# DaehwanKimLab/centrifuge

Hardware: NVIDIA H100
Metric: reads/sec (100 bp SE classification) (higher is better)
Workload: dtype u64

## Files before the change

centrifuge_b200/capi.py:

```python
import ctypes as C
import os

import numpy as np

HERE = os.path.dirname(os.path.abspath(__file__))
LIB_PATH = os.path.join(HERE, "libcfb200.so")

CFB_UID_NONE = 0xFFFFFFFF
REC_DTYPE = np.dtype([("taxid", "<u8"), ("score", "<u4"), ("hitlen", "<u4"), ("uid", "<u4"), ("pad", "<u4")])

_lib = None


class CfbError(RuntimeError):
    pass


class IndexInfo(C.Structure):
    _fields_ = [("len", C.c_uint64), ("num_sides", C.c_uint64), ("n_seqs", C.c_uint64), ("n_tax_nodes", C.c_uint64),
                ("n_boundaries", C.c_uint64), ("line_rate", C.c_int32), ("off_rate", C.c_int32), ("ftab_chars", C.c_int32),
                ("sample_bytes", C.c_int32), ("compressed", C.c_int32), ("device", C.c_int32), ("device_bytes", C.c_uint64)]


class IndexTables(C.Structure):
# ... 289 lines not shown

    def search_iter_stats(self):
        out = (C.c_uint64 * 8)()
        _ck(lib().cfb_ctx_search_iter_stats(self.h, out))
        names = ["warp_iters", "lane_requests", "consumer_paths", "restart_paths", "task_iters", "clk_head", "clk_wait", "clk_tail"]
        return dict(zip(names, [int(x) for x in out]))

    def score_stats(self):
        out = (C.c_uint64 * 23)()
        _ck(lib().cfb_ctx_score_stats(self.h, out))
        v = [int(x) for x in out]
        names = ["units", "rows", "distinct_ids", "reduce_units", "reduce_rounds", "warps", "warps_global"]
        d = dict(zip(names, v[:7]))
        d["rows_hist"], d["distinct_ids_hist"] = v[7:15], v[15:23]
        return d

    def long_stats(self):
        out = (C.c_uint64 * 4)()
        _ck(lib().cfb_ctx_long_stats(self.h, out))
        return dict(zip(["units", "bases", "segment_searches", "researched"], [int(x) for x in out]))

    def counters(self):
        out = (C.c_uint64 * 8)()
        _ck(lib().cfb_ctx_counters(self.h, out))
        names = ["units", "partial_searches", "ftab_probes", "sides_search", "walk_steps", "rows_resolved", "lf_steps", "ext_searches"]
        return dict(zip(names, [int(x) for x in out]))

    def launches(self):
        n = C.c_uint64()
        _ck(lib().cfb_ctx_kernel_launches(self.h, C.byref(n)))
# ... 253 lines not shown
```

centrifuge_b200/csrc/cf_logic.h:

```cpp
#ifndef CF_LOGIC_H_
#define CF_LOGIC_H_

#include <stdint.h>

#ifdef __CUDACC__
#define CFB_HD __host__ __device__ __forceinline__
#define CFB_HDN __host__ __device__
#else
#define CFB_HD inline
#define CFB_HDN inline
#endif

namespace cfb {

static const uint64_t kOff = 0xffffffffffffffffull;
static const uint64_t kUnk = 0xfffffffffffffffeull;
static const uint32_t kBwNone = 0xffffffffu;

struct alignas(16) SeqInfo {
	uint64_t taxid;
	int32_t  pid;
	uint32_t flags;
};
static const uint32_t kSeqExcluded = 1u;
// ... 30 lines not shown

struct Params {
	uint32_t khits, min_hitlen, ihits, increment;
	uint32_t tree_traverse, class_rank_slot;
};

struct HitRec { uint64_t top, bot; uint32_t bwoff, len; };

static const uint64_t kRowMask = (1ull << 40) - 1ull, kRowStart = 1ull << 63, kRowSameTs = 1ull << 58;

struct Counters {
	unsigned long long units, partial_searches, ftab_probes, sides_search, walk_steps, rows_resolved, lf_steps, ext_searches;
	unsigned long long req_rank16, req_ftab2, req_ftabk, req_walk8, req_ftabd;
	unsigned long long r16_w1, r16_w2_4, r16_w5, w8_try_row, w8_ok_row, w8_try_range, w8_ok_range, w8_ok_w5;
	unsigned long long it_warp, it_lane_req, it_consumers, it_restarts, it_task, clk_head, clk_wait, clk_tail;
	unsigned long long sc_units, sc_rows, sc_nmap, sc_reduce, sc_rounds, sc_warps, sc_warps_global;
	unsigned long long sc_rows_hist[8], sc_nmap_hist[8];
};

CFB_HD int popc64(uint64_t x) {
#ifdef __CUDA_ARCH__
	return __popcll(x);
#else
	return __builtin_popcountll(x);
#endif
}
CFB_HD uint32_t ctz32(uint32_t x) {
#ifdef __CUDA_ARCH__
	return (uint32_t)(__ffs(x) - 1);
#else
// ... 787 lines not shown
```

centrifuge_b200/csrc/cf_multi.cuh:

```cuda
#include <dlfcn.h>
#include <nccl.h>

extern "C" int cfb_ctx_count_records(cfb_ctx* c, int on) {
	if(!c) return fail(CFB_EINVAL, "null ctx");
	CK(cudaSetDevice(c->ix->device));
	if(on) { int rc = counts_init(c); if(rc) return rc; }
	c->fold_records = on != 0;
	return CFB_OK;
}
extern "C" int cfb_counts_taxids(cfb_ctx* c, uint64_t* taxid, uint64_t cap, uint64_t* n) {
	if(!c || !n) return fail(CFB_EINVAL, "null argument");
	CK(cudaSetDevice(c->ix->device));
	int rc = counts_init(c); if(rc) return rc;
	*n = c->cnt.n;
	if(taxid) { if(cap < c->cnt.n) return fail(CFB_EINVAL, "cfb_counts_taxids: buffer too small"); memcpy(taxid, c->cnt.h_taxid.data(), (size_t)c->cnt.n * 8); }
	return CFB_OK;
}
extern "C" int cfb_counts_reset(cfb_ctx* c) {
	if(!c) return fail(CFB_EINVAL, "null ctx");
	CK(cudaSetDevice(c->ix->device));
	if(!c->cnt.ready) return CFB_OK;
	CK(cudaDeviceSynchronize());
	CK(cudaMemset(c->cnt.total.p, 0, 3ull * c->cnt.n * 8)); CK(cudaMemset(c->cnt.global.p, 0, 3ull * c->cnt.n * 8));
	c->cnt.reduced = false;
// ... 153 lines not shown
	if(!c || !out) return fail(CFB_EINVAL, "null argument");
	CK(cudaSetDevice(c->ix->device));
	Counters h; CK(cudaMemcpy(&h, c->d_ctr, sizeof h, cudaMemcpyDeviceToHost));
	out[0] = h.it_warp; out[1] = h.it_lane_req; out[2] = h.it_consumers; out[3] = h.it_restarts; out[4] = h.it_task;
	out[5] = h.clk_head; out[6] = h.clk_wait; out[7] = h.clk_tail;
	return CFB_OK;
}
extern "C" int cfb_ctx_score_stats(cfb_ctx* c, uint64_t out[23]) {
	if(!c || !out) return fail(CFB_EINVAL, "null argument");
	CK(cudaSetDevice(c->ix->device));
	Counters h; CK(cudaMemcpy(&h, c->d_ctr, sizeof h, cudaMemcpyDeviceToHost));
	out[0] = h.sc_units; out[1] = h.sc_rows; out[2] = h.sc_nmap; out[3] = h.sc_reduce; out[4] = h.sc_rounds; out[5] = h.sc_warps; out[6] = h.sc_warps_global;
	for(int i = 0; i < 8; i++) { out[7 + i] = h.sc_rows_hist[i]; out[15 + i] = h.sc_nmap_hist[i]; }
	return CFB_OK;
}

__device__ __forceinline__ uint64_t gmix(uint64_t x) { x += 0x9E3779B97F4A7C15ull; x = (x ^ (x >> 30)) * 0xBF58476D1CE4E5B9ull; x = (x ^ (x >> 27)) * 0x94D049BB133111EBull; return x ^ (x >> 31); }
template <int W, int ILP>
__global__ void __launch_bounds__(128) k_gather_probe(const unsigned long long* __restrict__ a, uint64_t n, uint32_t iters, unsigned long long* sink) {
	const uint64_t tid = (uint64_t)blockIdx.x * blockDim.x + threadIdx.x;
	uint64_t h = gmix(tid * 0x2545F4914F6CDD1Dull + 1), acc = 0;
	for(uint32_t it = 0; it < iters; it++) {
		unsigned long long v[ILP][W];
		#pragma unroll
		for(int k = 0; k < ILP; k++) {
			h = gmix(h + k);
			const uint64_t u = h % n;
			if(W == 2) { const ulonglong2 q = __ldg(reinterpret_cast<const ulonglong2*>(a) + u); v[k][0] = q.x; v[k][W - 1] = q.y; }
			else v[k][0] = __ldg(a + u);
		}
// ... 42 lines not shown
```

centrifuge_b200/csrc/cfb200.cu:

```cuda
#include "../../include/cfb200.h"
#include "cf_index.h"
#include "cf_kernels.cuh"
#include <cub/cub.cuh>

#include <algorithm>
#include <atomic>
#include <mutex>
#include <thread>
#include <fcntl.h>
#include <unistd.h>
#include <cstdarg>
#include <cstdio>
#include <cstring>
#include <set>
#include <string>
#include <vector>

using namespace cfb;

enum { M_DONE = 0, M_FTAB = 1, M_LF = 2, M_NEED = 3, M_FTABK = 4, M_TASK = 5 };

struct SearchArgs {
	IndexView v; Params p; BatchView b;
	HitRec* hits; uint32_t* nhits; uint32_t cap;
// ... 557 lines not shown
		u.rdlen[r] = len; fw[r] = a.b.bases + a.b.off[m][unit]; tpos[r] = t0;
		const uint32_t raw[2] = {a.nhits[t0], a.nhits[t0 + 1]};
		for(int st = 0; st < 2; st++) {
			if(raw[st] & kListRegen) {
				const uint32_t slot = raw[st] & 0x3fffffffu;
				u.L[r][st] = a.regen + (size_t)slot * a.full_cap; u.n[r][st] = a.regen_n[slot]; found[r][st] = 0;
			} else {
				u.L[r][st] = a.hits + (t0 + st) * a.cap; u.n[r][st] = min(nh_stored(raw[st]), a.cap); found[r][st] = nh_found(raw[st]);
			}
		}
		for(int st = 0; st < 2; st++) if(list_dropped(raw, st)) u.n[r][st] = 0;
	}
	return u.n_mates > 0;
}

template <int MINB, bool EMIT_ONLY>
__global__ void __launch_bounds__(128, MINB) k_prep(const UnitArgs a) {
	const uint32_t unit = blockIdx.x * blockDim.x + threadIdx.x;
	const bool live = unit < a.b.n_units;
	UnitHits u; const uint8_t* fw[2]; uint32_t found[2][2]; size_t tpos[2];
	uint64_t rows = 0; bool have = false;
	if(live && (have = load_unit(a, unit, u, fw, found, tpos))) {
		if(EMIT_ONLY) { CountRows cr(a.p, u); for_each_visit(a.p, u, cr); rows = cr.rows; }
		else {
			Counters local; Counters* lc = nullptr;
			if(a.ctr) { memset(&local, 0, sizeof local); lc = &local; }
			if(!a.keep_short) for(int r = 0; r < u.n_mates; r++) {
				for(int st = 0; st < 2; st++) {
					if(!list_needs_regen(u.n[r][st], u.n[r][st ^ 1], found[r][st])) continue;
					const unsigned long long slot = atomicAdd(a.regen_ctr, 1ull);
					if(slot >= a.regen_slots) { atomicExch(a.overflow, 4u); continue; }
					HitRec* L = a.regen + (size_t)slot * a.full_cap;
					const uint32_t n = a.v.cr ? search_strand_dev<true>(a.v, a.p, fw[r], u.rdlen[r], st, L, a.full_cap)
					                          : search_strand_dev<false>(a.v, a.p, fw[r], u.rdlen[r], st, L, a.full_cap);
					if(n > a.full_cap) atomicExch(a.overflow, 1u);
					u.L[r][st] = L; u.n[r][st] = min(n, a.full_cap);
					a.regen_n[slot] = u.n[r][st]; a.nhits[tpos[r] + st] = kListRegen | (uint32_t)slot;
				}
			}
			for(int r = 0; r < u.n_mates; r++) {
				for(int st = 0; st < 2; st++) {
					if(!list_needs_exact_ranges(a.p, u.L[r][st], u.n[r][st], u.n[r][st ^ 1])) continue;
					for(uint32_t i = 0; i < u.n[r][st]; i++) {
						HitRec& h = u.L[r][st][i];
						if(h.top != kUnk) continue;
						HitRec t; uint32_t nc; bool dn;
						partial_search_scalar(a.v, fw[r], u.rdlen[r], st, h.bwoff, t, nc, dn, nullptr);
						h.top = t.top; h.bot = t.bot;
					}
				}
			}
			for(int r = 0; r < u.n_mates; r++) post_search(a.v, a.p, fw[r], u.rdlen[r], u.L[r][0], u.n[r][0], u.L[r][1], u.n[r][1], lc);
			SortAndCount sc(a.p, u);
			for_each_visit(a.p, u, sc);
// ... 3 lines not shown
				if(local.ext_searches) {
					atomicAdd(&a.ctr->ext_searches, local.ext_searches); atomicAdd(&a.ctr->partial_searches, local.partial_searches);
					atomicAdd(&a.ctr->ftab_probes, local.ftab_probes); atomicAdd(&a.ctr->sides_search, local.sides_search); atomicAdd(&a.ctr->lf_steps, local.lf_steps);
				}
			}
		}
		if(rows > 0xFFFFFFFFull) rows = 0xFFFFFFFFull;
	}
	const unsigned lane = threadIdx.x & 31;
	uint64_t incl = rows;
	for(int d = 1; d < 32; d <<= 1) { const uint64_t t = __shfl_up_sync(0xffffffffu, incl, d); if((int)lane >= d) incl += t; }
	const uint64_t warp_total = __shfl_sync(0xffffffffu, incl, 31);
	unsigned long long base = 0;
	if(lane == 31 && warp_total) base = atomicAdd(a.row_total, (unsigned long long)warp_total);
	base = __shfl_sync(0xffffffffu, base, 31);
	if(!live) return;
	const uint64_t off = base + incl - rows;
	a.nrows[unit] = (uint32_t)rows; a.row_off[unit] = off;
	if(rows && off + rows <= a.rows_cap) { EmitRows er(a.p, u, a.rows + off); for_each_visit(a.p, u, er); }
}

static const int kScoreThreads = 128;
static const uint32_t kScorePool = 232;
static const uint32_t kNoSlot = 0xffffffffu;
__device__ __forceinline__ uint32_t log2_bucket(uint64_t x) { const uint32_t b = 63u - (uint32_t)__clzll((long long)x); return b < 7u ? b : 7u; }
template <int MINB, bool COUNT>
__global__ void __launch_bounds__(kScoreThreads, MINB) k_score(const UnitArgs a) {
	__shared__ Entry s_map[kScorePool];
	__shared__ uint32_t s_used;
	if(threadIdx.x == 0) s_used = 0;
	__syncthreads();
	const uint32_t unit = blockIdx.x * blockDim.x + threadIdx.x;
	const unsigned lane = threadIdx.x & 31;
	const bool valid = unit < a.b.n_units;
// ... 159 lines not shown
			if(src < 0) break;
			chars |= (uint64_t)src << (2 * nv);
			row = next;
		}
		if(gl == 0) out[idx] = (row & kWalkRowMask) | (chars << 40) | ((uint64_t)nv << 56);
	}
}

__global__ void __launch_bounds__(256) k_lookup(const ResolveArgs a) {
	uint64_t n = *a.total; if(n > a.rows_cap) return;
	const uint64_t i = (uint64_t)blockIdx.x * blockDim.x + threadIdx.x;
	const uint64_t stride = (uint64_t)gridDim.x * blockDim.x;
	for(uint64_t k = i; k < n; k += stride) { const uint64_t r = a.rows[k] & kRowMask; a.ids[k] = a.v.rtab32 ? __ldg(a.v.rtab32 + r) : (uint32_t)__ldg(a.v.rtab16 + r); }
}

__global__ void __launch_bounds__(128) k_compact(uint32_t n_units, const uint64_t* row_off, const uint64_t* out_off,
                                                 const OutRec* sparse, OutRec* dense, uint32_t* rec_off32, uint64_t dense_cap, unsigned int* overflow) {
	const uint32_t unit = blockIdx.x * blockDim.x + threadIdx.x;
	if(unit > n_units) return;
	if(unit == n_units) { rec_off32[unit] = (uint32_t)out_off[unit]; return; }
	const uint64_t o = out_off[unit], n = out_off[unit + 1] - o;
	rec_off32[unit] = (uint32_t)o;
	if(o + n > dense_cap) { if(n) atomicExch(overflow, 3u); return; }
	const uint64_t src = row_off[unit];
	for(uint64_t i = 0; i < n; i++) dense[o + i] = sparse[src + i];
}

static const uint32_t kSegLen = 4096;
static_assert(kLongUnitLen == CFB_LONG_UNIT_LEN && kMaxMateLen == CFB_MAX_MATE_LEN, "cf_logic.h and cfb200.h disagree on the read length limits");
struct LongTask { uint64_t hoff, soff; uint32_t unit, mate, len, nseg; };
struct LongUnit { uint32_t unit, task0, ntask, pad; };
struct LongArgs {
	IndexView v; Params p; BatchView b;
	const LongTask* tasks; uint32_t ntasks; const LongUnit* units; uint32_t nunits; uint64_t nsegs;
	HitRec* seg; uint32_t* sn; uint32_t* sexit;
	HitRec* hits; uint32_t* nh;
	uint32_t* nrows; uint64_t* roff; uint32_t* hl;
	unsigned long long* stats;
	UnitArgs u;
};
// ... 385 lines not shown
}
extern "C" void cfb_params_default(cfb_params* p) {
	if(!p) return;
	memset(p, 0, sizeof *p); p->khits = 5; p->min_hitlen = 22; p->tree_traverse = 1; p->class_rank_slot = 0;
}

static const int kSlots = 17;

struct Slot {
	cudaStream_t st = nullptr;
	cudaEvent_t ev[6] = {nullptr, nullptr, nullptr, nullptr, nullptr, nullptr};
	HBuf<uint8_t> h_bases; HBuf<uint64_t> h_off; HBuf<uint32_t> h_len; HBuf<uint8_t> h_flags;
	DBuf<uint8_t> d_bases; DBuf<uint64_t> d_off; DBuf<uint32_t> d_len; DBuf<uint8_t> d_flags;
	HBuf<uint64_t> h_words; DBuf<uint64_t> d_words, d_npos, d_woff; DBuf<uint32_t> d_wlen;
	DBuf<uint64_t> pk; DBuf<uint32_t> nm;
	DBuf<HitRec> hits; DBuf<uint32_t> nhits; DBuf<HitRec> regen; DBuf<uint32_t> regen_n; uint64_t regen_slots = 0; uint32_t full_cap = 0; DBuf<uint32_t> nrows; DBuf<uint64_t> row_off; DBuf<uint64_t> bsum;
	DBuf<uint64_t> rows; DBuf<uint32_t> ids; DBuf<Entry> entries; DBuf<TaxCnt> tcs; DBuf<OutRec> sparse;
	DBuf<uint32_t> nout; DBuf<uint64_t> out_off; DBuf<uint8_t> scan_tmp; DBuf<OutRec> dense; DBuf<uint32_t> rec_off32;
	DBuf<unsigned long long> scal;
	HBuf<unsigned long long> h_scal;
	HBuf<OutRec> h_recs; HBuf<uint32_t> h_rec_off;
	DBuf<unsigned long long> cnt;
	bool folded = false, is_text = false, commit_pending = false;
	BatchView bv; uint64_t n_units = 0, n_bases = 0; uint32_t maxlen = 0, cap = 0; uint64_t rows_cap = 0, dense_cap = 0;
	bool pending = false, reran = false;
	bool want_host = false; uint64_t d2h_recs = 0;
	struct LongH { uint64_t unit; uint32_t len[2]; uint8_t fl; };
	std::vector<LongH> longs; uint64_t win_first = 0; uint32_t nlong_win = 0;
	HBuf<LongTask> h_ltask; HBuf<LongUnit> h_lunit; DBuf<LongTask> d_ltask; DBuf<LongUnit> d_lunit;
	DBuf<HitRec> lseg, lhits; DBuf<uint32_t> lsn, lsexit, lnh, lnrows, lhl; DBuf<uint64_t> lroff; DBuf<uint8_t> flags_short; DBuf<unsigned long long> lstats;
	uint64_t lhit_slots = 0, lsegs = 0; uint32_t lntasks = 0, lmaxlen = 0;
	void release() {
		h_bases.release(); h_off.release(); h_len.release(); h_flags.release(); d_bases.release(); d_off.release(); d_len.release(); d_flags.release();
		h_words.release(); d_words.release(); d_npos.release(); d_woff.release(); d_wlen.release();
		pk.release(); nm.release(); hits.release(); nhits.release(); regen.release(); regen_n.release(); nrows.release(); row_off.release(); bsum.release(); rows.release(); ids.release(); entries.release(); tcs.release();
		sparse.release(); nout.release(); out_off.release(); scan_tmp.release(); dense.release(); rec_off32.release(); scal.release(); h_scal.release(); h_recs.release(); h_rec_off.release(); cnt.release();
		h_ltask.release(); h_lunit.release(); d_ltask.release(); d_lunit.release(); lseg.release(); lhits.release(); lsn.release(); lsexit.release(); lnh.release();
		lnrows.release(); lhl.release(); lroff.release(); flags_short.release(); lstats.release();
		for(int i = 0; i < 6; i++) if(ev[i]) cudaEventDestroy(ev[i]);
		if(st) cudaStreamDestroy(st);
	}
};

struct cfb_dbatch { int slot; uint64_t n_units; };
struct TextCtx;
static void text_release(cfb_ctx*);
static void comm_release(cfb_ctx*);

struct CountsCtx {
	bool ready = false;
	std::vector<uint64_t> h_taxid; DBuf<uint64_t> d_taxid; uint32_t n = 0;
	DBuf<unsigned long long> total, global; bool reduced = false;
	void release() { d_taxid.release(); total.release(); global.release(); }
};

struct cfb_ctx {
	const cfb_index* ix = nullptr;
	IndexView view; Params prm;
	DBuf<uint64_t> d_host; DBuf<SeqInfo> d_seqs;
	Slot slots[kSlots];
	Counters* d_ctr = nullptr; int count = 0;
	uint64_t launches = 0;
	int resolve_blocks = 0;
	cfb_dbatch resident; bool resident_used = false;
	double rec_ratio = 2.0;
	uint64_t rows_cap0 = 0;
	TextCtx* text = nullptr;
	CountsCtx cnt; bool fold_records = false;
// ... 92 lines not shown
	*out = c;
	return CFB_OK;
}
extern "C" int cfb_ctx_slots(const cfb_ctx*) { return kSlots - 1; }
extern "C" int cfb_ctx_kernel_launches(const cfb_ctx* c, uint64_t* n) { if(!c || !n) return CFB_EINVAL; *n = c->launches; return CFB_OK; }

static int counts_init(cfb_ctx* c) {
	CountsCtx& k = c->cnt;
	if(k.ready) return CFB_OK;
	const HostIndex& h = c->ix->h;
	std::set<uint64_t> sp; sp.insert(0); sp.insert(1);
	for(size_t i = 0; i < h.nodes.size(); i++) sp.insert(h.nodes[i].taxid);
	sp.insert(h.seq_taxid.begin(), h.seq_taxid.end());
	k.h_taxid.assign(sp.begin(), sp.end()); k.n = (uint32_t)k.h_taxid.size();
	CK(k.d_taxid.ensure(k.n + 1)); CK(cudaMemcpy(k.d_taxid.p, k.h_taxid.data(), (size_t)k.n * 8, cudaMemcpyHostToDevice));
	CK(k.total.ensure(3ull * k.n)); CK(cudaMemset(k.total.p, 0, 3ull * k.n * 8));
	CK(k.global.ensure(3ull * k.n)); CK(cudaMemset(k.global.p, 0, 3ull * k.n * 8));
	k.ready = true;
	return CFB_OK;
}

struct FoldArgs {
	const uint64_t* sp_taxid; uint32_t n_sp;
	const uint32_t* rec_off; const OutRec* recs; uint32_t n_units; int32_t n_mates; uint32_t khits;
	const uint32_t* len[2]; const uint8_t* flags;
	unsigned long long* sp;
};
__device__ __forceinline__ int find_slot(const uint64_t* a, uint32_t n, uint64_t key) {
	uint32_t lo = 0, hi = n;
	while(lo < hi) { const uint32_t mid = (lo + hi) >> 1; if(a[mid] < key) lo = mid + 1; else hi = mid; }
	return (lo < n && a[lo] == key) ? (int)lo : -1;
}
__global__ void __launch_bounds__(128) k_fold_counts(const FoldArgs a) {
	const uint32_t u = blockIdx.x * 128 + threadIdx.x;
	const bool live = u < a.n_units;
	int first_slot = -1; uint32_t num = 1; bool qualifies = false;
	if(live) {
		const uint32_t r0 = a.rec_off[u], r1 = a.rec_off[u + 1];
		if(r1 == r0) { first_slot = find_slot(a.sp_taxid, a.n_sp, 0); qualifies = true; }
		else {
			uint32_t best = 0, ties = 0;
			for(uint32_t k = r0; k < r1; k++) { const uint32_t sc = a.recs[k].score; if(sc > best || k == r0) { best = sc; ties = 1; } else if(sc == best) ties++; }
			num = ties < a.khits ? ties : a.khits;
			const uint32_t fl = a.flags ? a.flags[u] : 3u;
			int64_t max_score = 0;
			if(fl & 1u) { const int64_t L = a.len[0][u]; max_score += L > 15 ? (L - 15) * (L - 15) : 0; }
			if(a.n_mates == 2 && (fl & 2u)) { const int64_t L = a.len[1][u]; max_score += L > 15 ? (L - 15) * (L - 15) : 0; }
			qualifies = (int64_t)best >= max_score;
			uint32_t taken = 0;
			for(uint32_t k = r0; k < r1 && taken < num; k++) {
				if(a.recs[k].score != best) continue;
				const int slot = find_slot(a.sp_taxid, a.n_sp, a.recs[k].taxid);
				if(taken == 0) first_slot = slot; else if(slot >= 0) atomicAdd(a.sp + slot, 1ull);
				taken++;
			}
		}
	}
	const int key = live ? first_slot : -1;
	const uint32_t peers = __match_any_sync(0xffffffffu, key);
	if(key >= 0) {
		const uint32_t uniq = __popc(__ballot_sync(peers, num == 1) & peers);
		const uint32_t obs = __popc(__ballot_sync(peers, num == 1 && qualifies) & peers);
		if((uint32_t)(__ffs(peers) - 1) == (threadIdx.x & 31u)) {
			atomicAdd(a.sp + key, (unsigned long long)__popc(peers));
			if(uniq) atomicAdd(a.sp + a.n_sp + key, (unsigned long long)uniq);
			if(obs) atomicAdd(a.sp + 2ull * a.n_sp + key, (unsigned long long)obs);
		}
	}
}
__global__ void k_cnt_commit(const unsigned long long* slot_sp, unsigned long long* total, uint32_t n) {
	const uint32_t i = blockIdx.x * blockDim.x + threadIdx.x;
	if(i < n) { const unsigned long long v = slot_sp[i]; if(v) atomicAdd(total + i, v); }
}

static int long_oom(const Slot& s, cudaError_t e, const char* what) {
	cudaGetLastError();
	uint64_t bases = 0; uint32_t mx = 0;
	for(const Slot::LongH& l : s.longs) { bases += (uint64_t)l.len[0] + l.len[1]; mx = std::max(mx, std::max(l.len[0], l.len[1])); }
	return fail(CFB_ENOMEM, "no device memory for %s of a batch with %zu long units (%llu bases, the longest read %u bases): %s", what,
	            s.longs.size(), (unsigned long long)bases, mx, cudaGetErrorString(e));
}
#define CKL(call, what) do { cudaError_t e_ = (call); if(e_ != cudaSuccess) { if(!s.longs.empty()) return long_oom(s, e_, what); CK(e_); } } while(0)

static int mate_too_long(uint64_t n, int m, const uint32_t* L) {
// ... 192 lines not shown
	BatchView sb = s.bv;
	if(s.nlong_win) sb.flags = s.flags_short.p;
	const uint32_t ublocks = (uint32_t)((n + 127) / 128);
	const uint64_t scan_blocks = (n + kScanBlock * kScanPer - 1) / (kScanBlock * kScanPer);
	if(n == 0) return CFB_OK;
	const SearchKernel search = search_kernel(s.maxlen, c->count, c->view.cr != nullptr);
	const bool keep_short = search == k_search_long<true> || search == k_search_long<false> || search == k_search_long<false, true> || c->prm.min_hitlen < kLongLen || c->keep_short;
	if(stage == 0) {
		if(s.cap == 0) {
			s.full_cap = s.maxlen / 4 + 8;
			s.cap = keep_short ? s.full_cap : s.maxlen / kLongLen + 2;
		}
		CK(s.hits.ensure(ntasks * s.cap)); CK(s.nhits.ensure(ntasks));
		if(!keep_short) {
			s.regen_slots = std::max<uint64_t>(s.regen_slots, c->regen_slots0 ? c->regen_slots0 : std::max<uint64_t>(ntasks / 32, 1024));
			CK(s.regen.ensure(s.regen_slots * s.full_cap)); CK(s.regen_n.ensure(s.regen_slots));
			CK(cudaMemsetAsync(s.scal.p + 6, 0, sizeof(unsigned long long), s.st));
		}
		const uint32_t W = (s.maxlen + 31) / 32 + 1;
		CK(s.pk.ensure(ntasks * W + 2)); CK(s.nm.ensure(ntasks * W + 2)); CK(s.nrows.ensure(n)); CK(s.row_off.ensure(n + 1));
		CK(s.bsum.ensure(scan_blocks + 1)); CK(s.nout.ensure(n + 1)); CK(s.out_off.ensure(n + 1)); CK(s.rec_off32.ensure(n + 1));
		s.rows_cap = std::max<uint64_t>(s.rows_cap, c->rows_cap0 ? c->rows_cap0 : std::max<uint64_t>(n * 12, 4096));
	}
	if(s.nlong_win) {
		CKL(s.rows.ensure(s.rows_cap), "the rows"); CKL(s.ids.ensure(s.rows_cap), "the rows"); CKL(s.entries.ensure(s.rows_cap), "the hit maps");
		CKL(s.tcs.ensure(s.rows_cap), "the hit maps"); CKL(s.sparse.ensure(s.rows_cap), "the records"); CKL(s.dense.ensure(s.rows_cap), "the records");
		CKL(s.lhl.ensure(s.rows_cap), "the rows");
	}
	CK(s.rows.ensure(s.rows_cap)); CK(s.ids.ensure(s.rows_cap)); CK(s.entries.ensure(s.rows_cap)); CK(s.tcs.ensure(s.rows_cap)); CK(s.sparse.ensure(s.rows_cap));
	s.dense_cap = s.rows_cap; CK(s.dense.ensure(s.dense_cap));
	CK(cudaMemsetAsync(s.scal.p, 0, 4 * sizeof(unsigned long long), s.st));
// ... 13 lines not shown
		SearchArgs sa; sa.v = c->view; sa.p = c->prm; sa.b = sb; sa.hits = s.hits.p; sa.nhits = s.nhits.p; sa.cap = s.cap;
		const uint32_t W = (s.maxlen + 31) / 32 + 1;
		sa.pk = s.pk.p; sa.nm = s.nm.p; sa.W = W; sa.keep_short = keep_short ? 1u : 0u;
		{ PackArgs pa; pa.b = sb; pa.pk = s.pk.p; pa.nm = s.nm.p; pa.W = W;
		  k_pack<<<(unsigned)((ntasks * W + 127) / 128), 128, 0, s.st>>>(pa); c->launches++; }
		sa.task_ctr64 = s.scal.p + 0; sa.ntasks = (uint32_t)ntasks; sa.overflow = (unsigned int*)(s.scal.p + 2); sa.ctr = ctr;
		int occ = 1;
		CK(cudaOccupancyMaxActiveBlocksPerMultiprocessor(&occ, search, kSearchThreads, 0));
		const uint64_t resident = (uint64_t)c->ix->sm_count * (uint64_t)std::max(occ, 1);
		const uint64_t warps = resident * (kSearchThreads / 32);
		sa.chunk = (uint32_t)std::min<uint64_t>(std::max<uint64_t>(ntasks / (warps * 4), 32), 256);
		const int blocks = (int)std::min<uint64_t>(resident, (ntasks + kSearchThreads - 1) / kSearchThreads);
		search<<<blocks, kSearchThreads, 0, s.st>>>(sa);
		c->launches++;
		if(time_it) CK(cudaEventRecord(s.ev[1], s.st));
		k_prep<8, false><<<ublocks, 128, 0, s.st>>>(ua); c->launches++;
	} else {
		if(time_it) CK(cudaEventRecord(s.ev[1], s.st));
		k_prep<8, true><<<ublocks, 128, 0, s.st>>>(ua); c->launches++;
	}
	LongArgs la;
	if(s.nlong_win) {
		la.v = c->view; la.p = c->prm; la.b = s.bv; la.tasks = s.d_ltask.p; la.ntasks = s.lntasks; la.units = s.d_lunit.p; la.nunits = s.nlong_win;
		la.nsegs = s.lsegs; la.seg = s.lseg.p; la.sn = s.lsn.p; la.sexit = s.lsexit.p; la.hits = s.lhits.p; la.nh = s.lnh.p;
		la.nrows = s.lnrows.p; la.roff = s.lroff.p; la.hl = s.lhl.p; la.stats = s.lstats.p; la.u = ua;
		const unsigned ub = (s.nlong_win + 31) / 32;
		if(stage == 0) {
			if(s.lntasks) {
				if(c->count == 1) k_long_join<true><<<(2 * s.lntasks + 127) / 128, 128, 0, s.st>>>(la);
				else {
// ... 13 lines not shown
	if((c->view.rtab16 || c->view.rtab32) && c->count != 1) k_lookup<<<c->ix->sm_count * 8, 256, 0, s.st>>>(ra);
	else if(c->view.cr) { if(c->count) k_resolve_c<true, false, true><<<c->resolve_blocks, kSearchThreads, 0, s.st>>>(ra); else k_resolve_c<false, false, true><<<c->resolve_blocks, kSearchThreads, 0, s.st>>>(ra); }
	else if(c->count) k_resolve_c<true, false><<<c->resolve_blocks, kSearchThreads, 0, s.st>>>(ra);
	else k_resolve_c<false, false><<<c->resolve_blocks, kSearchThreads, 0, s.st>>>(ra);
	c->launches++;
	if(time_it) CK(cudaEventRecord(s.ev[3], s.st));
	if(ctr) k_score<12, true><<<ublocks, kScoreThreads, 0, s.st>>>(ua);
	else k_score<12, false><<<ublocks, kScoreThreads, 0, s.st>>>(ua);
	if(s.nlong_win) { k_long_score<<<(s.nlong_win + 127) / 128, 128, 0, s.st>>>(la); c->launches++; }
	size_t scan_bytes = 0;
	CK(cub::DeviceScan::ExclusiveScan(nullptr, scan_bytes, s.nout.p, s.out_off.p, cub::Sum(), (uint64_t)0, (int)(n + 1), s.st));
	CK(s.scan_tmp.ensure(scan_bytes));
	CK(cudaMemsetAsync(s.nout.p + n, 0, sizeof(uint32_t), s.st));
	CK(cub::DeviceScan::ExclusiveScan(s.scan_tmp.p, scan_bytes, s.nout.p, s.out_off.p, cub::Sum(), (uint64_t)0, (int)(n + 1), s.st));
	CK(cudaMemcpyAsync(s.scal.p + 4, s.out_off.p + n, sizeof(uint64_t), cudaMemcpyDeviceToDevice, s.st));
	k_compact<<<(unsigned)((n + 1 + 127) / 128), 128, 0, s.st>>>((uint32_t)n, s.row_off.p, s.out_off.p, s.sparse.p, s.dense.p, s.rec_off32.p, s.dense_cap, (unsigned int*)(s.scal.p + 2));
	c->launches += 4;
	s.folded = false;
	if(c->fold_records && !s.is_text) {
		const uint32_t nsp = c->cnt.n;
		CK(s.cnt.ensure(3ull * nsp)); CK(cudaMemsetAsync(s.cnt.p, 0, 3ull * nsp * 8, s.st));
		FoldArgs fa; fa.sp_taxid = c->cnt.d_taxid.p; fa.n_sp = nsp; fa.rec_off = s.rec_off32.p; fa.recs = s.dense.p; fa.n_units = (uint32_t)n; fa.n_mates = nm;
		fa.khits = c->prm.khits; fa.len[0] = s.bv.len[0]; fa.len[1] = s.bv.len[1]; fa.flags = s.bv.flags; fa.sp = s.cnt.p;
		k_fold_counts<<<ublocks, 128, 0, s.st>>>(fa); c->launches++;
		s.folded = true;
	}
	if(time_it) CK(cudaEventRecord(s.ev[4], s.st));
	s.d2h_recs = 0;
	if(s.want_host) {
		const uint64_t guess = std::min<uint64_t>(s.dense_cap, (uint64_t)((double)n * c->rec_ratio * 1.05) + 4096);
		CK(s.h_recs.ensure(guess + 1)); CK(s.h_rec_off.ensure(n + 1));
		CK(cudaMemcpyAsync(s.h_rec_off.p, s.rec_off32.p, (n + 1) * 4, cudaMemcpyDeviceToHost, s.st));
		CK(cudaMemcpyAsync(s.h_recs.p, s.dense.p, guess * sizeof(OutRec), cudaMemcpyDeviceToHost, s.st));
		s.d2h_recs = guess;
	}
	CK(cudaMemcpyAsync(s.h_scal.p, s.scal.p, 8 * sizeof(unsigned long long), cudaMemcpyDeviceToHost, s.st));
	CK(cudaGetLastError());
	return CFB_OK;
}

static int finish_batch(cfb_ctx* c, Slot& s, bool time_it, bool to_host, cfb_result* out) {
// ... 198 lines not shown
```

include/cfb200.h:

```cpp
#ifndef CFB200_H_
#define CFB200_H_

#include <stddef.h>
#include <stdint.h>

#ifdef __cplusplus
extern "C" {
#endif

#define CFB_OK        0
#define CFB_EINVAL   -1
#define CFB_EIO      -2
#define CFB_ENOMEM   -3
#define CFB_ENODEV   -4
#define CFB_ECUDA    -5
#define CFB_EFORMAT  -6
#define CFB_EDATA    -7

#define CFB_UID_NONE 0xFFFFFFFFu

typedef struct cfb_index cfb_index;
typedef struct cfb_ctx   cfb_ctx;

int cfb_index_load(const char* basename, int device, cfb_index** out);
// ... 121 lines not shown
int cfb_counts_read(cfb_ctx*, int global, uint64_t* taxid, uint64_t* n_reads, uint64_t* n_unique, uint64_t* n_obs1, uint64_t cap, uint64_t* n);
int cfb_counts_dense(cfb_ctx*, int global, uint64_t* out, uint64_t cap);
#define CFB_COMM_ID_BYTES 128
int cfb_comm_unique_id(uint8_t id[CFB_COMM_ID_BYTES]);
int cfb_comm_init_rank(cfb_ctx*, int nranks, int rank, const uint8_t id[CFB_COMM_ID_BYTES]);
int cfb_comm_init_all(cfb_ctx* const* ctxs, int n);
int cfb_comm_info(const cfb_ctx*, int* rank, int* size, int* nccl_version);
int cfb_counts_allreduce(cfb_ctx* const* ctxs, int n, uint64_t* dense_out, uint64_t cap);

int cfb_ctx_requests(cfb_ctx*, uint64_t out[5]);
int cfb_ctx_request_breakdown(cfb_ctx*, uint64_t out[8]);
int cfb_gather_ceiling(const cfb_index*, int table, uint64_t n_requests, double* g_requests_per_s, double* ms);
int cfb_gather_rate(const cfb_index*, int table, uint64_t n_requests, int ctas_per_sm, int ilp, double* g_requests_per_s, double* ms);
int cfb_ctx_search_iter_stats(cfb_ctx*, uint64_t out[8]);
int cfb_ctx_score_stats(cfb_ctx*, uint64_t out[23]);

int cfb_ctx_counters(cfb_ctx*, uint64_t out[8]);
int cfb_ctx_long_stats(const cfb_ctx*, uint64_t out[4]);
int cfb_ctx_kernel_launches(const cfb_ctx*, uint64_t* n);

int   cfb_device_count(void);
void* cfb_host_alloc(size_t bytes);
void  cfb_host_free(void*);

int cfb_test_lf(const cfb_index*, const uint64_t* rows, const uint8_t* chars, uint64_t n, uint64_t* out);
int cfb_test_resolve(const cfb_index*, const uint64_t* rows, uint64_t n, uint32_t* out);
int cfb_test_parse(const char* path, int fasta, int trim5, int trim3, uint32_t seed, const char* out_path);
int cfb_test_host_path(const char* index_base, const char* reads_a, const char* reads_b, int fasta, int khits, uint32_t seed,
                       int trim5, int trim3, const uint32_t* rec_off, const cfb_rec* recs, uint64_t n_units,
                       const char* out_tsv, const char* out_report, const char* out_kreport);
// ... 70 lines not shown
```

Before: 309.4 million.

## Move strand regeneration to warp-per-task kernels and fold counts into compaction

Regeneration searches that used to run inline per thread inside k_prep now go through a planning kernel that compacts regen tasks with a warp prefix scan, followed by a grid-stride kernel where each task is handled by lane 0 of a warp. This is meant to remove the divergence of a few threads doing long searches while the rest of their warp waits. The separate count-folding kernel is merged into k_compact, and a per-sequence slot table avoids the binary search over taxids. Prep timing counters are also added. The costs are two extra launches and a regen path that appears to drop the compressed-index (cr) variant of the search.

```diff
diff --git a/centrifuge_b200/capi.py b/centrifuge_b200/capi.py
--- a/centrifuge_b200/capi.py
+++ b/centrifuge_b200/capi.py
@@ -327,6 +327,11 @@
         d = dict(zip(names, v[:7]))
         d["rows_hist"], d["distinct_ids_hist"] = v[7:15], v[15:23]
         return d
+
+    def prep_stats(self):
+        out = (C.c_uint64 * 4)()
+        _ck(lib().cfb_ctx_prep_stats(self.h, out))
+        return dict(zip(["regen_lists", "warps", "clk_all", "clk_regen"], [int(x) for x in out]))
 
     def long_stats(self):
         out = (C.c_uint64 * 4)()
diff --git a/centrifuge_b200/csrc/cf_logic.h b/centrifuge_b200/csrc/cf_logic.h
--- a/centrifuge_b200/csrc/cf_logic.h
+++ b/centrifuge_b200/csrc/cf_logic.h
@@ -68,6 +68,7 @@
 	unsigned long long req_rank16, req_ftab2, req_ftabk, req_walk8, req_ftabd;
 	unsigned long long r16_w1, r16_w2_4, r16_w5, w8_try_row, w8_ok_row, w8_try_range, w8_ok_range, w8_ok_w5;
 	unsigned long long it_warp, it_lane_req, it_consumers, it_restarts, it_task, clk_head, clk_wait, clk_tail;
+	unsigned long long pr_regen, pr_warps, pr_clk_all, pr_clk_regen;
 	unsigned long long sc_units, sc_rows, sc_nmap, sc_reduce, sc_rounds, sc_warps, sc_warps_global;
 	unsigned long long sc_rows_hist[8], sc_nmap_hist[8];
 };
diff --git a/centrifuge_b200/csrc/cf_multi.cuh b/centrifuge_b200/csrc/cf_multi.cuh
--- a/centrifuge_b200/csrc/cf_multi.cuh
+++ b/centrifuge_b200/csrc/cf_multi.cuh
@@ -191,6 +191,13 @@
 	for(int i = 0; i < 8; i++) { out[7 + i] = h.sc_rows_hist[i]; out[15 + i] = h.sc_nmap_hist[i]; }
 	return CFB_OK;
 }
+extern "C" int cfb_ctx_prep_stats(cfb_ctx* c, uint64_t out[4]) {
+	if(!c || !out) return fail(CFB_EINVAL, "null argument");
+	CK(cudaSetDevice(c->ix->device));
+	Counters h; CK(cudaMemcpy(&h, c->d_ctr, sizeof h, cudaMemcpyDeviceToHost));
+	out[0] = h.pr_regen; out[1] = h.pr_warps; out[2] = h.pr_clk_all; out[3] = h.pr_clk_regen;
+	return CFB_OK;
+}
 
 __device__ __forceinline__ uint64_t gmix(uint64_t x) { x += 0x9E3779B97F4A7C15ull; x = (x ^ (x >> 30)) * 0xBF58476D1CE4E5B9ull; x = (x ^ (x >> 27)) * 0x94D049BB133111EBull; return x ^ (x >> 31); }
 template <int W, int ILP>
diff --git a/centrifuge_b200/csrc/cfb200.cu b/centrifuge_b200/csrc/cfb200.cu
--- a/centrifuge_b200/csrc/cfb200.cu
+++ b/centrifuge_b200/csrc/cfb200.cu
@@ -595,30 +595,68 @@
 	return u.n_mates > 0;
 }
 
+__global__ void __launch_bounds__(128) k_regen_plan(const UnitArgs a, uint32_t* regen_task) {
+	const uint32_t unit = blockIdx.x * blockDim.x + threadIdx.x;
+	const unsigned lane = threadIdx.x & 31;
+	uint32_t want = 0;
+	if(unit < a.b.n_units) {
+		const uint8_t fl = a.b.flags ? a.b.flags[unit] : 3;
+		for(int m = 0; m < a.b.n_mates; m++) {
+			if(!((fl >> m) & 1) || a.b.len[m][unit] == 0) continue;
+			const size_t t0 = ((size_t)unit * a.b.n_mates + m) * 2;
+			const uint32_t raw[2] = {a.nhits[t0], a.nhits[t0 + 1]};
+			uint32_t n[2];
+			for(int st = 0; st < 2; st++) n[st] = list_dropped(raw, st) ? 0u : min(nh_stored(raw[st]), a.cap);
+			for(int st = 0; st < 2; st++) if(list_needs_regen(n[st], n[st ^ 1], nh_found(raw[st]))) want |= 1u << (2 * m + st);
+		}
+	}
+	const uint32_t cnt = __popc(want);
+	uint32_t incl = cnt;
+	for(int d = 1; d < 32; d <<= 1) { const uint32_t t = __shfl_up_sync(0xffffffffu, incl, d); if((int)lane >= d) incl += t; }
+	unsigned long long base = 0;
+	if(lane == 31 && incl) base = atomicAdd(a.regen_ctr, (unsigned long long)incl);
+	base = __shfl_sync(0xffffffffu, base, 31) + incl - cnt;
+	if(a.ctr && cnt) atomicAdd(&a.ctr->pr_regen, (unsigned long long)cnt);
+	for(; want; want &= want - 1) {
+		const int bit = __ffs(want) - 1, m = bit >> 1, st = bit & 1;
+		const size_t t0 = ((size_t)unit * a.b.n_mates + m) * 2;
+		const unsigned long long slot = base++;
+		if(slot >= a.regen_slots) { atomicExch(a.overflow, 4u); continue; }
+		regen_task[slot] = (uint32_t)(t0 + st);
+		a.nhits[t0 + st] = kListRegen | (uint32_t)slot;
+		const uint32_t other = a.nhits[t0 + (st ^ 1)];
+		if(!(other & kListRegen) && (other & kListNoLong)) a.nhits[t0 + (st ^ 1)] = 0;
+	}
+}
+__global__ void __launch_bounds__(128) k_regen(const UnitArgs a, const uint32_t* regen_task) {
+	const long long clk0 = a.ctr ? clock64() : 0;
+	const uint64_t n = min((uint64_t)*a.regen_ctr, a.regen_slots);
+	const uint64_t w0 = ((uint64_t)blockIdx.x * blockDim.x + threadIdx.x) >> 5, nw = ((uint64_t)gridDim.x * blockDim.x) >> 5;
+	if(threadIdx.x & 31) return;
+	for(uint64_t s = w0; s < n; s += nw) {
+		const uint32_t t = regen_task[s], st = t & 1u, mt = t >> 1;
+		const uint32_t unit = mt / (uint32_t)a.b.n_mates, m = mt - unit * (uint32_t)a.b.n_mates;
+		HitRec* L = a.regen + s * a.full_cap;
+		const uint32_t found = search_strand_dev<false>(a.v, a.p, a.b.bases + a.b.off[m][unit], a.b.len[m][unit], (int)st, L, a.full_cap);
+		if(found > a.full_cap) atomicExch(a.overflow, 1u);
+		a.regen_n[s] = min(found, a.full_cap);
+	}
+	if(a.ctr && w0 < n)
+		atomicAdd(&a.ctr->pr_clk_regen, (unsigned long long)(clock64() - clk0));
+}
+
 template <int MINB, bool EMIT_ONLY>
 __global__ void __launch_bounds__(128, MINB) k_prep(const UnitArgs a) {
 	const uint32_t unit = blockIdx.x * blockDim.x + threadIdx.x;
 	const bool live = unit < a.b.n_units;
 	UnitHits u; const uint8_t* fw[2]; uint32_t found[2][2]; size_t tpos[2];
 	uint64_t rows = 0; bool have = false;
+	const long long clk0 = !EMIT_ONLY && a.ctr ? clock64() : 0;
 	if(live && (have = load_unit(a, unit, u, fw, found, tpos))) {
 		if(EMIT_ONLY) { CountRows cr(a.p, u); for_each_visit(a.p, u, cr); rows = cr.rows; }
 		else {
 			Counters local; Counters* lc = nullptr;
 			if(a.ctr) { memset(&local, 0, sizeof local); lc = &local; }
-			if(!a.keep_short) for(int r = 0; r < u.n_mates; r++) {
-				for(int st = 0; st < 2; st++) {
-					if(!list_needs_regen(u.n[r][st], u.n[r][st ^ 1], found[r][st])) continue;
-					const unsigned long long slot = atomicAdd(a.regen_ctr, 1ull);
-					if(slot >= a.regen_slots) { atomicExch(a.overflow, 4u); continue; }
-					HitRec* L = a.regen + (size_t)slot * a.full_cap;
-					const uint32_t n = a.v.cr ? search_strand_dev<true>(a.v, a.p, fw[r], u.rdlen[r], st, L, a.full_cap)
-					                          : search_strand_dev<false>(a.v, a.p, fw[r], u.rdlen[r], st, L, a.full_cap);
-					if(n > a.full_cap) atomicExch(a.overflow, 1u);
-					u.L[r][st] = L; u.n[r][st] = min(n, a.full_cap);
-					a.regen_n[slot] = u.n[r][st]; a.nhits[tpos[r] + st] = kListRegen | (uint32_t)slot;
-				}
-			}
 			for(int r = 0; r < u.n_mates; r++) {
 				for(int st = 0; st < 2; st++) {
 					if(!list_needs_exact_ranges(a.p, u.L[r][st], u.n[r][st], u.n[r][st ^ 1])) continue;
@@ -652,10 +690,14 @@
 	unsigned long long base = 0;
 	if(lane == 31 && warp_total) base = atomicAdd(a.row_total, (unsigned long long)warp_total);
 	base = __shfl_sync(0xffffffffu, base, 31);
-	if(!live) return;
-	const uint64_t off = base + incl - rows;
-	a.nrows[unit] = (uint32_t)rows; a.row_off[unit] = off;
-	if(rows && off + rows <= a.rows_cap) { EmitRows er(a.p, u, a.rows + off); for_each_visit(a.p, u, er); }
+	if(live) {
+		const uint64_t off = base + incl - rows;
+		a.nrows[unit] = (uint32_t)rows; a.row_off[unit] = off;
+		if(rows && off + rows <= a.rows_cap) { EmitRows er(a.p, u, a.rows + off); for_each_visit(a.p, u, er); }
+	}
+	if(!EMIT_ONLY && a.ctr && __any_sync(0xffffffffu, live) && lane == 0) {
+		atomicAdd(&a.ctr->pr_warps, 1ull); atomicAdd(&a.ctr->pr_clk_all, (unsigned long long)(clock64() - clk0));
+	}
 }
 
 static const int kScoreThreads = 128;
@@ -845,16 +887,70 @@
 	for(uint64_t k = i; k < n; k += stride) { const uint64_t r = a.rows[k] & kRowMask; a.ids[k] = a.v.rtab32 ? __ldg(a.v.rtab32 + r) : (uint32_t)__ldg(a.v.rtab16 + r); }
 }
 
+struct alignas(16) SeqSlot { uint64_t taxid; uint32_t slot, pad; };
+struct FoldArgs {
+	const uint64_t* sp_taxid; uint32_t n_sp; int32_t n_mates; uint32_t khits;
+	const SeqSlot* seq_slot; uint32_t n_seqs;
+	const uint32_t* len[2]; const uint8_t* flags;
+	unsigned long long* sp;
+};
+__device__ __forceinline__ int find_slot(const uint64_t* a, uint32_t n, uint64_t key) {
+	uint32_t lo = 0, hi = n;
+	while(lo < hi) { const uint32_t mid = (lo + hi) >> 1; if(a[mid] < key) lo = mid + 1; else hi = mid; }
+	return (lo < n && a[lo] == key) ? (int)lo : -1;
+}
 __global__ void __launch_bounds__(128) k_compact(uint32_t n_units, const uint64_t* row_off, const uint64_t* out_off,
-                                                 const OutRec* sparse, OutRec* dense, uint32_t* rec_off32, uint64_t dense_cap, unsigned int* overflow) {
+                                                 const OutRec* sparse, OutRec* dense, uint32_t* rec_off32, uint64_t dense_cap, unsigned int* overflow,
+                                                 const FoldArgs f) {
 	const uint32_t unit = blockIdx.x * blockDim.x + threadIdx.x;
-	if(unit > n_units) return;
-	if(unit == n_units) { rec_off32[unit] = (uint32_t)out_off[unit]; return; }
-	const uint64_t o = out_off[unit], n = out_off[unit + 1] - o;
-	rec_off32[unit] = (uint32_t)o;
-	if(o + n > dense_cap) { if(n) atomicExch(overflow, 3u); return; }
-	const uint64_t src = row_off[unit];
-	for(uint64_t i = 0; i < n; i++) dense[o + i] = sparse[src + i];
+	const bool live = unit < n_units;
+	if(unit == n_units) rec_off32[unit] = (uint32_t)out_off[unit];
+	int first_slot = -1; uint32_t num = 1; bool qualifies = false;
+	if(live) {
+		const uint64_t o = out_off[unit], n = out_off[unit + 1] - o;
+		rec_off32[unit] = (uint32_t)o;
+		const bool fits = o + n <= dense_cap;
+		if(!fits && n) atomicExch(overflow, 3u);
+		const uint64_t src = row_off[unit];
+		uint32_t best = 0, ties = 0;
+		for(uint64_t i = 0; i < n; i++) {
+			const OutRec r = sparse[src + i];
+			if(r.score > best || i == 0) { best = r.score; ties = 1; } else if(r.score == best) ties++;
+			if(fits) dense[o + i] = r;
+		}
+		if(f.sp && n == 0) { first_slot = 0; qualifies = true; }
+		else if(f.sp) {
+			num = ties < f.khits ? ties : f.khits;
+			const uint32_t fl = f.flags ? f.flags[unit] : 3u;
+			int64_t max_score = 0;
+			if(fl & 1u) { const int64_t L = f.len[0][unit]; max_score += L > 15 ? (L - 15) * (L - 15) : 0; }
+			if(f.n_mates == 2 && (fl & 2u)) { const int64_t L = f.len[1][unit]; max_score += L > 15 ? (L - 15) * (L - 15) : 0; }
+			qualifies = (int64_t)best >= max_score;
+			uint32_t taken = 0;
+			for(uint64_t i = 0; i < n && taken < num; i++) {
+				const OutRec& r = sparse[src + i];
+				if(r.score != best) continue;
+				int slot;
+				const SeqSlot q = r.uid < f.n_seqs ? f.seq_slot[r.uid] : SeqSlot{~0ull, kNoSlot, 0};
+				if(r.uid < f.n_seqs && q.taxid == r.taxid) slot = q.slot == kNoSlot ? -1 : (int)q.slot;
+				else slot = find_slot(f.sp_taxid, f.n_sp, r.taxid);
+				if(taken == 0) first_slot = slot; else if(slot >= 0) atomicAdd(f.sp + slot, 1ull);
+				taken++;
+			}
+		}
+	}
+	if(!f.sp) return;
+	const int key = live ? first_slot : -1;
+	const uint32_t peers = __match_any_sync(0xffffffffu, key);
+	if(key >= 0) {
+		const uint32_t uniq = __popc(__ballot_sync(peers, num == 1) & peers);
+		const uint32_t obs = __popc(__ballot_sync(peers, num == 1 && qualifies) & peers);
+		if((uint32_t)(__ffs(peers) - 1) == (threadIdx.x & 31u)) {
+			atomicAdd(f.sp + key, (unsigned long long)__popc(peers));
+			if(uniq) atomicAdd(f.sp + f.n_sp + key, (unsigned long long)uniq);
+			if(obs) atomicAdd(f.sp + 2ull * f.n_sp + key, (unsigned long long)obs);
+		}
+	}
 }
 
 static const uint32_t kSegLen = 4096;
@@ -1270,7 +1366,7 @@
 	DBuf<uint8_t> d_bases; DBuf<uint64_t> d_off; DBuf<uint32_t> d_len; DBuf<uint8_t> d_flags;
 	HBuf<uint64_t> h_words; DBuf<uint64_t> d_words, d_npos, d_woff; DBuf<uint32_t> d_wlen;
 	DBuf<uint64_t> pk; DBuf<uint32_t> nm;
-	DBuf<HitRec> hits; DBuf<uint32_t> nhits; DBuf<HitRec> regen; DBuf<uint32_t> regen_n; uint64_t regen_slots = 0; uint32_t full_cap = 0; DBuf<uint32_t> nrows; DBuf<uint64_t> row_off; DBuf<uint64_t> bsum;
+	DBuf<HitRec> hits; DBuf<uint32_t> nhits; DBuf<HitRec> regen; DBuf<uint32_t> regen_n, regen_task; uint64_t regen_slots = 0; uint32_t full_cap = 0; DBuf<uint32_t> nrows; DBuf<uint64_t> row_off; DBuf<uint64_t> bsum;
 	DBuf<uint64_t> rows; DBuf<uint32_t> ids; DBuf<Entry> entries; DBuf<TaxCnt> tcs; DBuf<OutRec> sparse;
 	DBuf<uint32_t> nout; DBuf<uint64_t> out_off; DBuf<uint8_t> scan_tmp; DBuf<OutRec> dense; DBuf<uint32_t> rec_off32;
 	DBuf<unsigned long long> scal;
@@ -1289,7 +1385,7 @@
 	void release() {
 		h_bases.release(); h_off.release(); h_len.release(); h_flags.release(); d_bases.release(); d_off.release(); d_len.release(); d_flags.release();
 		h_words.release(); d_words.release(); d_npos.release(); d_woff.release(); d_wlen.release();
-		pk.release(); nm.release(); hits.release(); nhits.release(); regen.release(); regen_n.release(); nrows.release(); row_off.release(); bsum.release(); rows.release(); ids.release(); entries.release(); tcs.release();
+		pk.release(); nm.release(); hits.release(); nhits.release(); regen.release(); regen_n.release(); regen_task.release(); nrows.release(); row_off.release(); bsum.release(); rows.release(); ids.release(); entries.release(); tcs.release();
 		sparse.release(); nout.release(); out_off.release(); scan_tmp.release(); dense.release(); rec_off32.release(); scal.release(); h_scal.release(); h_recs.release(); h_rec_off.release(); cnt.release();
 		h_ltask.release(); h_lunit.release(); d_ltask.release(); d_lunit.release(); lseg.release(); lhits.release(); lsn.release(); lsexit.release(); lnh.release();
 		lnrows.release(); lhl.release(); lroff.release(); flags_short.release(); lstats.release();
@@ -1306,8 +1402,9 @@
 struct CountsCtx {
 	bool ready = false;
 	std::vector<uint64_t> h_taxid; DBuf<uint64_t> d_taxid; uint32_t n = 0;
+	DBuf<SeqSlot> seq_slot; uint32_t n_seqs = 0;
 	DBuf<unsigned long long> total, global; bool reduced = false;
-	void release() { d_taxid.release(); total.release(); global.release(); }
+	void release() { d_taxid.release(); seq_slot.release(); total.release(); global.release(); }
 };
 
 struct cfb_ctx {
@@ -1430,60 +1527,24 @@
 	sp.insert(h.seq_taxid.begin(), h.seq_taxid.end());
 	k.h_taxid.assign(sp.begin(), sp.end()); k.n = (uint32_t)k.h_taxid.size();
 	CK(k.d_taxid.ensure(k.n + 1)); CK(cudaMemcpy(k.d_taxid.p, k.h_taxid.data(), (size_t)k.n * 8, cudaMemcpyHostToDevice));
+	{
+		const size_t ns = h.seq_taxid.size();
+		std::vector<SeqInfo> si(ns); std::vector<SeqSlot> ss(ns + 1);
+		if(ns) CK(cudaMemcpy(si.data(), c->d_seqs.p, ns * sizeof(SeqInfo), cudaMemcpyDeviceToHost));
+		for(size_t i = 0; i < ns; i++) {
+			const auto it = std::lower_bound(k.h_taxid.begin(), k.h_taxid.end(), si[i].taxid);
+			ss[i].taxid = si[i].taxid; ss[i].pad = 0;
+			ss[i].slot = it != k.h_taxid.end() && *it == si[i].taxid ? (uint32_t)(it - k.h_taxid.begin()) : kNoSlot;
+		}
+		CK(k.seq_slot.ensure(ns + 1)); CK(cudaMemcpy(k.seq_slot.p, ss.data(), ns * sizeof(SeqSlot), cudaMemcpyHostToDevice));
+		k.n_seqs = (uint32_t)ns;
+	}
 	CK(k.total.ensure(3ull * k.n)); CK(cudaMemset(k.total.p, 0, 3ull * k.n * 8));
 	CK(k.global.ensure(3ull * k.n)); CK(cudaMemset(k.global.p, 0, 3ull * k.n * 8));
 	k.ready = true;
 	return CFB_OK;
 }
 
-struct FoldArgs {
-	const uint64_t* sp_taxid; uint32_t n_sp;
-	const uint32_t* rec_off; const OutRec* recs; uint32_t n_units; int32_t n_mates; uint32_t khits;
-	const uint32_t* len[2]; const uint8_t* flags;
-	unsigned long long* sp;
-};
-__device__ __forceinline__ int find_slot(const uint64_t* a, uint32_t n, uint64_t key) {
-	uint32_t lo = 0, hi = n;
-	while(lo < hi) { const uint32_t mid = (lo + hi) >> 1; if(a[mid] < key) lo = mid + 1; else hi = mid; }
-	return (lo < n && a[lo] == key) ? (int)lo : -1;
-}
-__global__ void __launch_bounds__(128) k_fold_counts(const FoldArgs a) {
-	const uint32_t u = blockIdx.x * 128 + threadIdx.x;
-	const bool live = u < a.n_units;
-	int first_slot = -1; uint32_t num = 1; bool qualifies = false;
-	if(live) {
-		const uint32_t r0 = a.rec_off[u], r1 = a.rec_off[u + 1];
-		if(r1 == r0) { first_slot = find_slot(a.sp_taxid, a.n_sp, 0); qualifies = true; }
-		else {
-			uint32_t best = 0, ties = 0;
-			for(uint32_t k = r0; k < r1; k++) { const uint32_t sc = a.recs[k].score; if(sc > best || k == r0) { best = sc; ties = 1; } else if(sc == best) ties++; }
-			num = ties < a.khits ? ties : a.khits;
-			const uint32_t fl = a.flags ? a.flags[u] : 3u;
-			int64_t max_score = 0;
-			if(fl & 1u) { const int64_t L = a.len[0][u]; max_score += L > 15 ? (L - 15) * (L - 15) : 0; }
-			if(a.n_mates == 2 && (fl & 2u)) { const int64_t L = a.len[1][u]; max_score += L > 15 ? (L - 15) * (L - 15) : 0; }
-			qualifies = (int64_t)best >= max_score;
-			uint32_t taken = 0;
-			for(uint32_t k = r0; k < r1 && taken < num; k++) {
-				if(a.recs[k].score != best) continue;
-				const int slot = find_slot(a.sp_taxid, a.n_sp, a.recs[k].taxid);
-				if(taken == 0) first_slot = slot; else if(slot >= 0) atomicAdd(a.sp + slot, 1ull);
-				taken++;
-			}
-		}
-	}
-	const int key = live ? first_slot : -1;
-	const uint32_t peers = __match_any_sync(0xffffffffu, key);
-	if(key >= 0) {
-		const uint32_t uniq = __popc(__ballot_sync(peers, num == 1) & peers);
-		const uint32_t obs = __popc(__ballot_sync(peers, num == 1 && qualifies) & peers);
-		if((uint32_t)(__ffs(peers) - 1) == (threadIdx.x & 31u)) {
-			atomicAdd(a.sp + key, (unsigned long long)__popc(peers));
-			if(uniq) atomicAdd(a.sp + a.n_sp + key, (unsigned long long)uniq);
-			if(obs) atomicAdd(a.sp + 2ull * a.n_sp + key, (unsigned long long)obs);
-		}
-	}
-}
 __global__ void k_cnt_commit(const unsigned long long* slot_sp, unsigned long long* total, uint32_t n) {
 	const uint32_t i = blockIdx.x * blockDim.x + threadIdx.x;
 	if(i < n) { const unsigned long long v = slot_sp[i]; if(v) atomicAdd(total + i, v); }
@@ -1706,7 +1767,7 @@
 		CK(s.hits.ensure(ntasks * s.cap)); CK(s.nhits.ensure(ntasks));
 		if(!keep_short) {
 			s.regen_slots = std::max<uint64_t>(s.regen_slots, c->regen_slots0 ? c->regen_slots0 : std::max<uint64_t>(ntasks / 32, 1024));
-			CK(s.regen.ensure(s.regen_slots * s.full_cap)); CK(s.regen_n.ensure(s.regen_slots));
+			CK(s.regen.ensure(s.regen_slots * s.full_cap)); CK(s.regen_n.ensure(s.regen_slots)); CK(s.regen_task.ensure(s.regen_slots));
 			CK(cudaMemsetAsync(s.scal.p + 6, 0, sizeof(unsigned long long), s.st));
 		}
 		const uint32_t W = (s.maxlen + 31) / 32 + 1;
@@ -1750,6 +1811,11 @@
 		search<<<blocks, kSearchThreads, 0, s.st>>>(sa);
 		c->launches++;
 		if(time_it) CK(cudaEventRecord(s.ev[1], s.st));
+		if(!keep_short) {
+			k_regen_plan<<<ublocks, 128, 0, s.st>>>(ua, s.regen_task.p);
+			k_regen<<<c->ix->sm_count * 16, 128, 0, s.st>>>(ua, s.regen_task.p);
+			c->launches += 2;
+		}
 		k_prep<8, false><<<ublocks, 128, 0, s.st>>>(ua); c->launches++;
 	} else {
 		if(time_it) CK(cudaEventRecord(s.ev[1], s.st));
@@ -1793,17 +1859,16 @@
 	CK(cudaMemsetAsync(s.nout.p + n, 0, sizeof(uint32_t), s.st));
 	CK(cub::DeviceScan::ExclusiveScan(s.scan_tmp.p, scan_bytes, s.nout.p, s.out_off.p, cub::Sum(), (uint64_t)0, (int)(n + 1), s.st));
 	CK(cudaMemcpyAsync(s.scal.p + 4, s.out_off.p + n, sizeof(uint64_t), cudaMemcpyDeviceToDevice, s.st));
-	k_compact<<<(unsigned)((n + 1 + 127) / 128), 128, 0, s.st>>>((uint32_t)n, s.row_off.p, s.out_off.p, s.sparse.p, s.dense.p, s.rec_off32.p, s.dense_cap, (unsigned int*)(s.scal.p + 2));
+	const bool fold = c->fold_records && !s.is_text;
+	FoldArgs fa; memset(&fa, 0, sizeof fa);
+	if(fold) {
+		CK(s.cnt.ensure(3ull * c->cnt.n)); CK(cudaMemsetAsync(s.cnt.p, 0, 3ull * c->cnt.n * 8, s.st));
+		fa.sp_taxid = c->cnt.d_taxid.p; fa.n_sp = c->cnt.n; fa.n_mates = nm; fa.seq_slot = c->cnt.seq_slot.p; fa.n_seqs = c->cnt.n_seqs;
+		fa.khits = c->prm.khits; fa.len[0] = s.bv.len[0]; fa.len[1] = s.bv.len[1]; fa.flags = s.bv.flags; fa.sp = s.cnt.p;
+	}
+	k_compact<<<(unsigned)((n + 1 + 127) / 128), 128, 0, s.st>>>((uint32_t)n, s.row_off.p, s.out_off.p, s.sparse.p, s.dense.p, s.rec_off32.p, s.dense_cap, (unsigned int*)(s.scal.p + 2), fa);
 	c->launches += 4;
-	s.folded = false;
-	if(c->fold_records && !s.is_text) {
-		const uint32_t nsp = c->cnt.n;
-		CK(s.cnt.ensure(3ull * nsp)); CK(cudaMemsetAsync(s.cnt.p, 0, 3ull * nsp * 8, s.st));
-		FoldArgs fa; fa.sp_taxid = c->cnt.d_taxid.p; fa.n_sp = nsp; fa.rec_off = s.rec_off32.p; fa.recs = s.dense.p; fa.n_units = (uint32_t)n; fa.n_mates = nm;
-		fa.khits = c->prm.khits; fa.len[0] = s.bv.len[0]; fa.len[1] = s.bv.len[1]; fa.flags = s.bv.flags; fa.sp = s.cnt.p;
-		k_fold_counts<<<ublocks, 128, 0, s.st>>>(fa); c->launches++;
-		s.folded = true;
-	}
+	s.folded = fold;
 	if(time_it) CK(cudaEventRecord(s.ev[4], s.st));
 	s.d2h_recs = 0;
 	if(s.want_host) {
diff --git a/include/cfb200.h b/include/cfb200.h
--- a/include/cfb200.h
+++ b/include/cfb200.h
@@ -159,6 +159,7 @@
 int cfb_gather_rate(const cfb_index*, int table, uint64_t n_requests, int ctas_per_sm, int ilp, double* g_requests_per_s, double* ms);
 int cfb_ctx_search_iter_stats(cfb_ctx*, uint64_t out[8]);
 int cfb_ctx_score_stats(cfb_ctx*, uint64_t out[23]);
+int cfb_ctx_prep_stats(cfb_ctx*, uint64_t out[4]);
 
 int cfb_ctx_counters(cfb_ctx*, uint64_t out[8]);
 int cfb_ctx_long_stats(const cfb_ctx*, uint64_t out[4]);
```

Result: faster. 314.7 million, median of 6 (+1.7%).
